# feifeibear/long-context-attention

Measured on AMD Instinct MI355X. Metric: attention TFLOP/s (algorithmic, causal fwd+bwd) + iter ms of LongContextAttention at seqlen 64K, ulysses x ring, higher is better.
Workload: dtype bf16

## Files before the change

long-context-attention_amd/csrc/usp_flash_bwd_dq64.hip:

```cpp
#include "usp_bwd_params.hpp"
#include "usp_host.hpp"
#include "usp_mfma64.hpp"

namespace usp {

#ifndef USP_Q64_PF
#define USP_Q64_PF 3
#endif
constexpr int kQ64_PF = USP_Q64_PF;
#ifndef USP_Q64_Y1
#define USP_Q64_Y1 24
#endif
constexpr int kQ64_Y1 = USP_Q64_Y1;

#ifdef USP_Q64_TIMING
#define USP_TM(...) __VA_ARGS__
#else
#define USP_TM(...)
#endif

template <int DT, bool CAUSAL>
__global__ __launch_bounds__(256, 1) void flash_bwd_dq64_kernel(const BwdParams ) {
  using E = Elem<DT>;
  using M = M64<DT>;
  constexpr int D = 128, kBM = 256;
  constexpr int ROWB = D * 2;
  constexpr int TILEB = kTile * ROWB;
  constexpr int VOFF = 2 * TILEB;
  constexpr int NKT = D / 16, NDJ = D / 32;
  constexpr int PF = kQ64_PF;

  extern __shared__ __attribute__((aligned(16))) char smem_raw[];
  if ((uint32_t)(uintptr_t)(USP_LDS char*)smem_raw != 0u) __builtin_trap();
  USP_LDS char* smem = (USP_LDS char*)(uintptr_t)0;

  const int tid = threadIdx.x;
  const int lane = tid & 63;
  const int wave = __builtin_amdgcn_readfirstlane(tid >> 6);
  const int l31 = lane & 31;
  const int hi = lane >> 5;
  typedef const __attribute__((address_space(4))) BwdParams* KArgs;
  KArgs p = (KArgs)__builtin_amdgcn_kernarg_segment_ptr();
  asm volatile("" : "+s"(p));

  const int dma_row = lane >> 4;
  const int dma_c8 = ((lane & 15) ^ ((lane >> 4) << 2)) * 16;
  const int k_voff = dma_row * (int)p->k_ss * 2 + dma_c8, v_voff = dma_row * (int)p->v_ss * 2 + dma_c8;
  const int rd_base = l31 * ROWB + ((hi ^ tile_swz<D>(l31)) * 16);
  int tr_addr[NDJ][2];
  {
    const int i = lane & 15, grp = (lane >> 4) & 1;
#pragma unroll
    for (int dj = 0; dj < NDJ; ++dj)
#pragma unroll
      for (int e = 0; e < 2; ++e) {
        const int rr = 8 * e + 4 * hi + (i >> 2);
        const int slot = 4 * dj + 2 * grp + ((i & 3) >> 1);
        tr_addr[dj][e] = rr * ROWB + ((slot ^ tile_swz<D>(rr)) * 16) + (i & 1) * 8;
      }
  }
  const float c = p->scale_log2;

  const ItemWalk walk(p->n_items);
  for (int pass = 0;; ++pass) {
  int w = walk.at(pass);
  if (w < 0) break;
  asm volatile("" : "+s"(p));
  USP_TM(const uint64_t tm_item = __builtin_amdgcn_s_memtime();)
  w = walk.dealt(w, p->nblk);
  if (p->ksplit <= 1) w = walk.grouped(w, p->nblk, p->walk_g);
  const int qt_r = w % p->nblk;
  int rest = w / p->nblk;
  const int qt = CAUSAL ? (p->nblk - 1 - qt_r) : qt_r;
  int cut = 0;
  if (p->ksplit > 1) { cut = rest % p->ksplit; rest /= p->ksplit; }
  const int h = rest % p->Hq, b = rest / p->Hq;
  const int hkv = h / p->G;
  const int q0 = qt * kBM;
  const int qw = q0 + wave * 64;
  const int off = p->causal_off;

  int blk_kv_end = p->Sk, wave_kv_end = p->Sk;
  if (CAUSAL) {
    const int blk_last = (q0 + kBM < p->Sq ? q0 + kBM : p->Sq) - 1;
    const int wav_last = (qw + 64 < p->Sq ? qw + 64 : p->Sq) - 1;
    blk_kv_end = blk_last + off + 1 < p->Sk ? blk_last + off + 1 : p->Sk;
    wave_kv_end = wav_last + off + 1 < p->Sk ? wav_last + off + 1 : p->Sk;
  }
  if (qw >= p->Sq) wave_kv_end = 0;
  const int nt = blk_kv_end > 0 ? (blk_kv_end + kTile - 1) / kTile : 0;
  int n_full = p->Sk / kTile;
// ... 31 lines not shown
                 "global_load_dwordx4 %12, %17, off offset:128\n\tglobal_load_dwordx4 %13, %17, off offset:160\n\t"
                 "global_load_dwordx4 %14, %17, off offset:192\n\tglobal_load_dwordx4 %15, %17, off offset:224\n\t"
                 "s_waitcnt vmcnt(0)"
                 : "=&a"(qf[qb][0]), "=&a"(qf[qb][1]), "=&a"(qf[qb][2]), "=&a"(qf[qb][3]), "=&a"(qf[qb][4]), "=&a"(qf[qb][5]),
                   "=&a"(qf[qb][6]), "=&a"(qf[qb][7]), "=&a"(df[qb][0]), "=&a"(df[qb][1]), "=&a"(df[qb][2]), "=&a"(df[qb][3]),
                   "=&a"(df[qb][4]), "=&a"(df[qb][5]), "=&a"(df[qb][6]), "=&a"(df[qb][7])
                 : "v"(qp), "v"(dp) : "memory");
#endif
    const float lse = p->lse[b * p->lse_sb + h * p->lse_sh + row_c];
    const float dlt = p->delta[b * p->dl_sb + h * p->dl_sh + row_c];
    const bool live = row < p->Sq && lse != USP_NEG_INF;
    nl[qb] = live ? -lse * kLog2e : USP_NEG_INF;
    dl[qb] = live ? dlt : 0.f;
  }

  const int k_rowb = (int)p->k_ss * 2, v_rowb = (int)p->v_ss * 2;
  const int64_t k_tb = (int64_t)kTile * k_rowb, v_tb = (int64_t)kTile * v_rowb;
  int k_step = 4 * k_rowb - 1024, v_step = 4 * v_rowb - 1024;
  int lds_w = wave * 4096;
  const char* k_cur = p->k + 2 * (b * p->k_sb + hkv * p->k_sh) + (int64_t)wave * 16 * k_rowb + tb * k_tb;
  const char* v_cur = p->v + 2 * (b * p->v_sb + hkv * p->v_sh) + (int64_t)wave * 16 * v_rowb + tb * v_tb;
  int rows_kv = p->Sk - 16 * wave - tb * kTile;
  u32x4 k_rs, v_rs;
  int dma_buf = 0;
  auto dma_open = [&](int buf) {
    k_rs = make_rsrc_rows(k_cur, rows_kv, 16, k_rowb, 2 * D);
    v_rs = make_rsrc_rows(v_cur, rows_kv, 16, v_rowb, 2 * D);
    dma_buf = buf;
    k_cur += k_tb;
    v_cur += v_tb;
    rows_kv -= kTile;
  };
  auto dma_piece = [&](int n) {
    asm volatile("" : "+s"(lds_w), "+s"(k_step), "+s"(v_step));
    const int i = n & 3;
    if (n < 4) lds_dma16_asm(k_rs, lds_w + dma_buf * TILEB, k_voff ^ (16 * i), i * k_step, i);
    else lds_dma16_asm(v_rs, lds_w + VOFF + dma_buf * TILEB, v_voff ^ (16 * i), i * v_step, i);
  };

  f32x16 dq[2][NDJ];
#pragma unroll
  for (int qb = 0; qb < 2; ++qb)
#pragma unroll
    for (int dj = 0; dj < NDJ; ++dj) {
#pragma unroll
      for (int r = 0; r < 16; ++r) dq[qb][dj][r] = 0.f;
      pin_agpr(dq[qb][dj]);
    }

  dma_open(tb & 1);
#pragma unroll
  for (int n = 0; n < 8; ++n) dma_piece(n);
  dma_drain();
  __syncthreads();

  auto iter = [&](auto mask_c, int t, bool work) __attribute__((always_inline)) {
    constexpr bool MASK = decltype(mask_c)::value;
    const int par = t & 1;
    if (work) {
#pragma unroll
      for (int qb = 0; qb < 2; ++qb)
#pragma unroll
        for (int kt = 0; kt < NKT; ++kt) { pin_agpr4(qf[qb][kt]); pin_agpr4(df[qb][kt]); }
      int kr = rd_base + par * TILEB, vr = rd_base + VOFF + par * TILEB;
      asm volatile("" : "+v"(kr), "+v"(vr));
      USP_LDS const char* kt_base = smem + par * TILEB;
      f32x16 bs[2][2], bd[2][2];
      u32x4 pk[2][4];
      u32x4 ka[2 * NKT], va[2 * NKT], xa[4 * NDJ];
      auto rd_k = [&](int f) { ka[f] = *(USP_LDS const u32x4*)(smem + (f & 1) * 32 * ROWB + (kr ^ (32 * (f >> 1)))); };
      auto rd_v = [&](int f) { va[f] = *(USP_LDS const u32x4*)(smem + (f & 1) * 32 * ROWB + (vr ^ (32 * (f >> 1)))); };
      auto rd_x = [&](int f) {
        USP_LDS const char* xb = kt_base + (f / NDJ) * 16 * ROWB;
        const u32x2 a0 = lds_read_tr16(xb + tr_addr[f % NDJ][0]);
        const u32x2 a1 = lds_read_tr16(xb + tr_addr[f % NDJ][1]);
        xa[f] = u32x4{a0[0], a0[1], a1[0], a1[1]};
      };
      auto X = [&](int qb, int n) {
        const int ks = n >> 3, kb = ks >> 1, r = 8 * (ks & 1) + (n & 7);
        bs[qb][kb][r] = fast_exp2(__builtin_fmaf(bs[qb][kb][r], c, nl[qb]));
      };
      auto Y = [&](int qb, int n) {
        const int ks = n >> 3, kb = ks >> 1, r = 8 * (ks & 1) + (n & 7);
        bd[qb][kb][r] = (bd[qb][kb][r] - dl[qb]) * bs[qb][kb][r];
        if (r & 1) pk[qb][ks][(n & 7) >> 1] = E::pack2(bd[qb][kb][r - 1], bd[qb][kb][r]);
      };
      auto mask = [&](int qb) {
        const int row = qw + 32 * qb + l31;
        int klim = p->Sk - 1;
        if (CAUSAL) klim = row + off < klim ? row + off : klim;
        const int kb0 = t * kTile + 4 * hi;
#pragma unroll
        for (int r = 0; r < 16; ++r) {
          const int key = kb0 + (r & 3) + 8 * (r >> 2);
          if (key > klim) bs[qb][0][r] = USP_NEG_INF;
          if (key + 32 > klim) bs[qb][1][r] = USP_NEG_INF;
        }
      };
#pragma unroll
      for (int f = 0; f < PF; ++f) rd_k(f);
      __builtin_amdgcn_sched_barrier(0);
#pragma unroll
      for (int i = 0; i < 16; ++i) {
        const int kt = i >> 1, kb = i & 1;
        if (kt == 0) M::template s_first<MASK>(bs[0][kb], ka[i], qf[0][0]);
        else M::template s_next<MASK>(bs[0][kb], ka[i], qf[0][kt]);
        if (i == 0) { __builtin_amdgcn_sched_barrier(0); dma_open(par ^ 1); }
        if (i + PF < 16) rd_k(i + PF);
        if (i >= 1 && i <= 8) dma_piece(i - 1);
        __builtin_amdgcn_sched_barrier(0);
      }
      if (MASK) { mfma_settle(bs[0]); mask(0); }
#pragma unroll
      for (int i = 0; i < 16; ++i) {
        const int kt = i >> 1, kb = i & 1;
        if (kt == 0) M::template s_first<MASK>(bs[1][kb], ka[i], qf[1][0]);
        else M::template s_next<MASK>(bs[1][kb], ka[i], qf[1][kt]);
        if (i == 0) __builtin_amdgcn_sched_barrier(0);
        X(0, 2 * i); X(0, 2 * i + 1);
        if (i >= 16 - PF) rd_v(i - (16 - PF));
        __builtin_amdgcn_sched_barrier(0);
      }
      if (MASK) { mfma_settle(bs[1]); mask(1); }
#pragma unroll
      for (int i = 0; i < 16; ++i) {
        const int kt = i >> 1, kb = i & 1;
        if (kt == 0) M::template s_first<MASK>(bd[0][kb], va[i], df[0][0]);
        else M::template s_next<MASK>(bd[0][kb], va[i], df[0][kt]);
        if (i == 0) __builtin_amdgcn_sched_barrier(0);
        if (i + PF < 16) rd_v(i + PF);
        X(1, 2 * i); X(1, 2 * i + 1);
        __builtin_amdgcn_sched_barrier(0);
      }
#pragma unroll
      for (int i = 0; i < 16; ++i) {
        const int kt = i >> 1, kb = i & 1;
        if (kt == 0) M::template s_first<MASK>(bd[1][kb], va[i], df[1][0]);
        else M::template s_next<MASK>(bd[1][kb], va[i], df[1][kt]);
        if (i == 0) __builtin_amdgcn_sched_barrier(0);
        Y(0, 2 * i); Y(0, 2 * i + 1);
        if (i >= 16 - PF) rd_x(i - (16 - PF));
        __builtin_amdgcn_sched_barrier(0);
      }
      constexpr int NY1 = kQ64_Y1;
      static_assert(NY1 >= 16 && NY1 <= 28, "dS of k-step ks must be packed before gap 16 + 4 ks");
#pragma unroll
      for (int i = 0; i < 16; ++i) {
        M::template o_acc<MASK>(dq[0][i % NDJ], xa[i], pk[0][i / NDJ]);
        if (i == 0) __builtin_amdgcn_sched_barrier(0);
        if (i + PF < 16) rd_x(i + PF);
#pragma unroll
        for (int n = i * 32 / NY1; n < (i + 1) * 32 / NY1; ++n) Y(1, n);
        __builtin_amdgcn_sched_barrier(0);
      }
#pragma unroll
      for (int i = 0; i < 16; ++i) {
        M::template o_acc<MASK>(dq[1][i % NDJ], xa[i], pk[1][i / NDJ]);
        if (16 + i < NY1) {
#pragma unroll
          for (int n = (16 + i) * 32 / NY1; n < (16 + i + 1) * 32 / NY1; ++n) Y(1, n);
        }
        __builtin_amdgcn_sched_barrier(0);
      }
    } else {
      dma_open(par ^ 1);
#pragma unroll
      for (int n = 0; n < 8; ++n) dma_piece(n);
    }
    dma_drain();
    __syncthreads();
  };
  const std::integral_constant<bool, false> plain;
  const std::integral_constant<bool, true> masked;
  int t = tb;
  USP_TM(const uint64_t tm_loop = __builtin_amdgcn_s_memtime();)
  __builtin_amdgcn_s_waitcnt(0x0f70);
  for (; t < e_full; ++t) iter(plain, t, true);
  __builtin_amdgcn_s_waitcnt(0x0f70);
  for (; t < e_own; ++t) iter(masked, t, true);
  mfma_settle(dq);
  USP_TM(const uint64_t tm_own = __builtin_amdgcn_s_memtime(); const uint64_t tm_plain_n = n_full;)
  for (; t < te; ++t) iter(plain, t, false);
  USP_TM(const uint64_t tm_epi = __builtin_amdgcn_s_memtime();)

  mfma_settle(dq);
  asm volatile("" : "+s"(p));
  const bool wide = (p->wide16 & 1) != 0;
#pragma unroll
  for (int qb = 0; qb < 2; ++qb) {
    const int row = qw + 32 * qb + l31;
    if (wide) {
      const int row_c = row < p->Sq ? row : 0;
      store_row16_wide<E, NDJ>(p->dq16 + 2 * (b * p->dq16_sb + (int64_t)row_c * p->dq16_ss + h * p->dq16_sh), dq[qb], p->scale, hi,
                               row < p->Sq);
    } else if (row < p->Sq) {
      float* o1 = p->dq + b * p->dq_sb + (int64_t)row * p->dq_ss + h * p->dq_sh;
      char* h1 = p->dq16 ? p->dq16 + 2 * (b * p->dq16_sb + (int64_t)row * p->dq16_ss + h * p->dq16_sh) : nullptr;
      int acc_f = p->accum_dq;
      if (p->ksplit > 1) {
        o1 = p->ws_dq + ((((int64_t)cut * p->B + b) * p->Sq + row) * p->Hq + h) * D;
        h1 = nullptr;
        acc_f = 0;
      }
      const float sc = p->scale;
#pragma unroll
      for (int dj = 0; dj < NDJ; ++dj)
#pragma unroll
        for (int g4 = 0; g4 < 4; ++g4) {
          const int d0 = 32 * dj + 8 * g4 + 4 * hi;
          f32x4 v1 = {dq[qb][dj][4 * g4] * sc, dq[qb][dj][4 * g4 + 1] * sc, dq[qb][dj][4 * g4 + 2] * sc,
                      dq[qb][dj][4 * g4 + 3] * sc};
          if (acc_f) v1 += *(const f32x4*)(o1 + d0);
          if (h1) *(u32x2*)(h1 + 2 * d0) = u32x2{E::pack2(v1[0], v1[1]), E::pack2(v1[2], v1[3])};
          else *(f32x4*)(o1 + d0) = v1;
        }
    }
  }
  __syncthreads();
USP_TM(
  if (pass < 3 && lane == 0 && (blockIdx.x % 61) == 0)
    printf("TQ wg %3d pass %d wave %d qt %2d tiles own %3d (plain %3d) wg %3d : prologue %6llu own tiles %8llu (%5llu / tile) idle %6llu epilogue %6llu\n",
           (int)blockIdx.x, pass, wave, qt, n_w, (int)tm_plain_n, nt, (unsigned long long)(tm_loop - tm_item),
           (unsigned long long)(tm_own - tm_loop), (unsigned long long)((tm_own - tm_loop) / (n_w > 0 ? n_w : 1)),
           (unsigned long long)(tm_epi - tm_own), (unsigned long long)(__builtin_amdgcn_s_memtime() - tm_epi));
)
  }
}

bool dq64_serves(const BwdParams& p_in) {
  if (p_in.seq_q || p_in.seq_k || p_in.sched || p_in.win_on) return false;
  if ((p_in.k_ss * 2) % 256 != 0 || (p_in.v_ss * 2) % 256 != 0 || p_in.k_ss * 128 >= (1LL << 31) || p_in.v_ss * 128 >= (1LL << 31))
    return false;
  return true;
}

bool launch_dq64(const BwdParams& p_in, int dtype, bool causal, hipStream_t st, int* rc) {
  if (!dq64_serves(p_in)) return false;
  BwdParams p = p_in;
  p.nblk = (p.Sq + 255) / 256;
  p.n_items = p.B * p.Hq * p.nblk * p.ksplit;
  p.wide16 = (p.ksplit <= 1 && p.dq16 && !p.accum_dq && tensor_aligned(p.dq16, p.dq16_sb, p.dq16_ss, p.dq16_sh, 16, 8)) ? 1 : 0;
  const int grid = persistent_grid(p.n_items, device_cus(), p.interleave);
  const size_t lds = 4 * kTile * 128 * 2;
  with_dtype_causal(dtype, causal, [&](auto dt, auto c) {
    hipLaunchKernelGGL((flash_bwd_dq64_kernel<decltype(dt)::value, decltype(c)::value>), dim3(grid), dim3(256), lds, st, p);
  });
  *rc = launched();
  return true;
}

}
```

long-context-attention_amd/csrc/usp_flash_fwd64.hip:

```cpp
#include "usp_fwd_params.hpp"
#include "usp_host.hpp"
#include "usp_mfma64.hpp"

namespace usp {

#ifndef USP_F64_NEA
#define USP_F64_NEA 42
#endif
constexpr int kF64_NEA = USP_F64_NEA;
#ifndef USP_F64_LEAD
#define USP_F64_LEAD 2
#endif
constexpr int kF64_LEAD = USP_F64_LEAD;
#ifndef USP_F64_PFK
#define USP_F64_PFK 2
#endif
constexpr int kF64_PFK = USP_F64_PFK;
#ifndef USP_F64_PFV
#define USP_F64_PFV 2
#endif
constexpr int kF64_PFV = USP_F64_PFV;
#ifndef USP_F64_MAX0
#define USP_F64_MAX0 22
#endif
constexpr int kF64_MAX0 = USP_F64_MAX0;
#ifndef USP_F64_DMA0
#define USP_F64_DMA0 2
#endif
constexpr int kF64_DMA0 = USP_F64_DMA0;
#ifndef USP_F64_DMAS
#define USP_F64_DMAS 6
#endif
constexpr int kF64_DMAS = USP_F64_DMAS;

#ifdef USP_F64_TIMING
#define USP_TM(...) __VA_ARGS__
#else
#define USP_TM(...)
#endif

template <int DT, bool CAUSAL, bool SPLIT = false>
__global__ __launch_bounds__(256, 1) void flash_fwd64_kernel(const FwdArgsT<SPLIT> ) {
  using E = Elem<DT>;
  using M = M64<DT>;
  constexpr int D = 128;
  constexpr int kBM = 256;
  constexpr int ROWB = D * 2;
  constexpr int KBYTES = kBN * ROWB;
  constexpr int NKT = D / 16;
  constexpr int NDJ = D / 32;
  constexpr int VOFF = 2 * KBYTES;

  extern __shared__ __attribute__((aligned(16))) char smem_raw[];
  USP_LDS char* smem = (USP_LDS char*)smem_raw;

  const int tid = threadIdx.x;
  const int lane = tid & 63;
  const int wave = __builtin_amdgcn_readfirstlane(tid >> 6);
  const int l31 = lane & 31;
  const int hi = lane >> 5;
  typedef const __attribute__((address_space(4))) FwdArgsT<SPLIT>* KArgs;
  KArgs p = (KArgs)__builtin_amdgcn_kernarg_segment_ptr();
  asm volatile("" : "+s"(p));

  const int k_voff = (16 * wave + (lane >> 4)) * (int)p->k_ss * 2 + (((lane & 15) ^ (lane >> 4)) * 16);
  const int v_voff = (16 * wave + ((lane & 15) >> 2)) * (int)p->v_ss * 2 + (32 * (lane >> 4) + 8 * (lane & 3)) * 2;
  const int k_rd = l31 * ROWB + ((hi ^ (l31 & 15)) * 16);
  const int v_rd = VOFF + hi * NDJ * 256 + ((lane & 15) >> 2) * 64 + ((lane >> 4) & 1) * 32 + (lane & 3) * 8;
  const float c = p->scale_log2;

  const ItemWalk walk(p->n_items);
  for (int pass = 0;; ++pass) {
  int w = walk.at(pass);
  if (w < 0) break;
// ... 32 lines not shown
    off -= kb;
  }
  auto n_keys = [&]() { if constexpr (SPLIT) return sk_cut; else return p->Sk; };

  int blk_kv_end = n_keys(), wave_kv_end = n_keys();
  if (CAUSAL) {
    const int blk_last = (q0 + kBM < p->Sq ? q0 + kBM : p->Sq) - 1;
    const int wav_last = (qw + 64 < p->Sq ? qw + 64 : p->Sq) - 1;
    blk_kv_end = blk_last + off + 1 < n_keys() ? blk_last + off + 1 : n_keys();
    wave_kv_end = wav_last + off + 1 < n_keys() ? wav_last + off + 1 : n_keys();
  }
  if (qw >= p->Sq) wave_kv_end = 0;
  const int nt = blk_kv_end > 0 ? (blk_kv_end + kBN - 1) / kBN : 0;
  int n_full = n_keys() / kBN;
  if (CAUSAL) {
    const int lim = qw + off + 1;
    const int nf = lim > 0 ? lim / kBN : 0;
    n_full = nf < n_full ? nf : n_full;
  }
  if (n_full > nt) n_full = nt;

USP_TM(
  const uint64_t tm_item = __builtin_amdgcn_s_memtime();
)
  u32x4 qf[2][NKT];
#pragma unroll
  for (int qb = 0; qb < 2; ++qb) {
    const int row = qw + 32 * qb + l31;
    const int row_c = row < p->Sq ? row : p->Sq - 1;
    const char* qp = p->q + 2 * (b * p->q_sb + (int64_t)row_c * p->q_ss + h * p->q_sh) + 16 * hi;
#pragma unroll
    for (int t = 0; t < NKT; ++t) qf[qb][t] = *(const u32x4*)(qp + 32 * t);
  }
#pragma unroll
  for (int qb = 0; qb < 2; ++qb)
#pragma unroll
    for (int t = 0; t < NKT; ++t) pin_agpr4(qf[qb][t]);

  const int64_t k_tb = (int64_t)kBN * p->k_ss * 2, v_tb = (int64_t)kBN * p->v_ss * 2;
  const char* k_cur = p->k + 2 * (b * p->k_sb + hkv * p->k_sh);
  const char* v_cur = p->v + 2 * (b * p->v_sb + hkv * p->v_sh);
  if constexpr (SPLIT) { k_cur += 2 * (int64_t)kb * p->k_ss; v_cur += 2 * (int64_t)kb * p->v_ss; }
  int rows_kv = n_keys();
  const int k_rowb = (int)p->k_ss * 2, v_rowb = (int)p->v_ss * 2;
  int lds_w = wave * 4096, k_step = 4 * (int)p->k_ss * 2 - 1024, v_step = 4 * (int)p->v_ss * 2 - 1024;
  u32x4 k_rs, v_rs;
  int k_ahead = 0;
  int dma_kbuf = 0, dma_vbuf = 0;
  auto dma_open = [&](int kbuf, int vbuf) {
    k_rs = make_rsrc_rows(k_cur, rows_kv + kBN * k_ahead, kBN, k_rowb, 2 * D);
    v_rs = make_rsrc_rows(v_cur, rows_kv, kBN, v_rowb, 2 * D);
    k_cur += k_tb;
    v_cur += v_tb;
    rows_kv -= kBN;
    dma_kbuf = kbuf; dma_vbuf = vbuf;
  };
  auto dma_open_k = [&](int kbuf) {
    k_rs = make_rsrc_rows(k_cur, rows_kv, kBN, k_rowb, 2 * D);
    k_cur += k_tb;
    k_ahead = -1;
    dma_kbuf = kbuf;
  };
  auto dma_piece = [&](int n) {
    asm volatile("" : "+s"(lds_w), "+s"(k_step), "+s"(v_step));
    if (n < 4) lds_dma16_asm(k_rs, lds_w + dma_kbuf * KBYTES, k_voff ^ (64 * n), n * k_step, n);
    else lds_dma16_asm(v_rs, lds_w + VOFF + dma_vbuf * KBYTES, v_voff, (n - 4) * v_step, n - 4);
  };
  auto dma_all = [&](int kbuf, int vbuf) {
    dma_open(kbuf, vbuf);
#pragma unroll
    for (int n = 0; n < 8; ++n) dma_piece(n);
  };

  f32x16 o[2][NDJ];
#pragma unroll
  for (int qb = 0; qb < 2; ++qb)
#pragma unroll
    for (int dj = 0; dj < NDJ; ++dj) {
#pragma unroll
      for (int r = 0; r < 16; ++r) o[qb][dj][r] = 0.f;
      pin_agpr(o[qb][dj]);
    }
  float m_run[2] = {USP_NEG_INF, USP_NEG_INF};
  float l_run[2] = {0.f, 0.f};

  auto qk = [&](int kbuf, f32x16 (&s)[2][2]) {
#pragma unroll
    for (int kt = 0; kt < NKT; ++kt) {
      USP_LDS const char* kp = smem + kbuf * KBYTES + (k_rd ^ (32 * kt));
      const u32x4 k0 = *(USP_LDS const u32x4*)kp;
      const u32x4 k1 = *(USP_LDS const u32x4*)(kp + 32 * ROWB);
#pragma unroll
      for (int qb = 0; qb < 2; ++qb) {
        if (kt == 0) { M::template s_first<true>(s[qb][0], k0, qf[qb][0]); M::template s_first<true>(s[qb][1], k1, qf[qb][0]); }
        else { M::template s_next<true>(s[qb][0], k0, qf[qb][kt]); M::template s_next<true>(s[qb][1], k1, qf[qb][kt]); }
      }
    }
    mfma_settle(s);
  };
  auto mask = [&](int kt0, f32x16 (&s)[2][2]) {
#pragma unroll
    for (int qb = 0; qb < 2; ++qb) {
      const int row = qw + 32 * qb + l31;
      int klim = n_keys() - 1;
      if (CAUSAL) klim = row + off < klim ? row + off : klim;
      const int kb0 = kt0 + 4 * hi;
#pragma unroll
      for (int r = 0; r < 16; ++r) {
        const int key = kb0 + (r & 3) + 8 * (r >> 2);
        if (key > klim) s[qb][0][r] = USP_NEG_INF;
        if (key + 32 > klim) s[qb][1][r] = USP_NEG_INF;
      }
    }
  };
  f32x16 sa[2][2], sb[2][2];
#pragma unroll
  for (int qb = 0; qb < 2; ++qb)
#pragma unroll
    for (int kb = 0; kb < 2; ++kb)
#pragma unroll
      for (int r = 0; r < 16; ++r) { sa[qb][kb][r] = 0.f; sb[qb][kb][r] = 0.f; }
  dma_all(0, 0);
  dma_open_k(1);
#pragma unroll
  for (int n = 0; n < 4; ++n) dma_piece(n);
  dma_drain();
  __syncthreads();
  if (nt > 0 && wave_kv_end > 0) qk(0, sa);
  __syncthreads();

  constexpr float kThr = 8.f;
  constexpr int NA = 32, NB = 32;
  constexpr int NEA = kF64_NEA, LEAD = kF64_LEAD, PFK = kF64_PFK, PFV = kF64_PFV, MAX0 = kF64_MAX0;
  constexpr int DMA0 = kF64_DMA0, DMAS = kF64_DMAS;
  static_assert(64 - NEA <= 22, "k-step 3 of P must be complete two slots before slot 24 of phase B");
  static_assert(MAX0 >= 1 && MAX0 < NB && DMAS >= 1 && DMA0 + 7 * DMAS < NA + NB, "");
  const float thr_raw = kThr / c;
  float m_thr[2] = {USP_NEG_INF, USP_NEG_INF};
  float nmc[2] = {0.f, 0.f};
  auto first_ref = [&](const float (&mt_lane)[2]) {
#pragma unroll
    for (int qb = 0; qb < 2; ++qb) {
      const float m_new = xhalf_max(mt_lane[qb]);
      const float m_use = (m_new == USP_NEG_INF) ? 0.f : m_new;
      m_run[qb] = m_new;
      m_thr[qb] = m_new + thr_raw;
      nmc[qb] = -(m_use * c);
    }
  };
  auto rescale = [&](const float (&mt_lane)[2]) {
    asm volatile("; rescale (rare)" ::: "memory");
    mfma_settle(o);
#pragma unroll
    for (int qb = 0; qb < 2; ++qb) {
      const float m_new = fmaxf(m_run[qb], xhalf_max(mt_lane[qb]));
      const float m_use = (m_new == USP_NEG_INF) ? 0.f : m_new;
// ... 9 lines not shown
    }
#pragma unroll
    for (int qb = 0; qb < 2; ++qb)
#pragma unroll
      for (int dj = 0; dj < NDJ; ++dj) pin_agpr(o[qb][dj]);
    operand_settle();
  };
  auto decide = [&](f32x16 (&s)[2][2]) {
    float mt[2];
#pragma unroll
    for (int qb = 0; qb < 2; ++qb) {
      mt[qb] = s[qb][0][0];
#pragma unroll
      for (int r = 1; r < 16; ++r) mt[qb] = fmaxf(mt[qb], s[qb][0][r]);
#pragma unroll
      for (int r = 0; r < 16; ++r) mt[qb] = fmaxf(mt[qb], s[qb][1][r]);
    }
    first_ref(mt);
  };
  auto iter = [&](auto par_c, auto mode_c, int jpar, int kt0_next, f32x16 (&cs)[2][2], f32x16 (&ns)[2][2])
      __attribute__((always_inline)) {
    constexpr int PARV = decltype(par_c)::value, MODE = decltype(mode_c)::value;
    const int par = PARV < 2 ? PARV : jpar;
    dma_open(par, par ^ 1);
    auto dma_slot = [&](int g) {
      if (g >= DMA0 && (g - DMA0) % DMAS == 0 && (g - DMA0) / DMAS < 8) dma_piece((g - DMA0) / DMAS);
    };
    USP_LDS const char* kb = smem + (par ^ 1) * KBYTES;
    USP_LDS const char* vb = smem + par * KBYTES + v_rd;
    int kr = k_rd;
    asm volatile("" : "+v"(kr));
    u32x4 ka[2 * NKT];
    auto rd_k = [&](int f) {
      ka[f] = *(USP_LDS const u32x4*)(kb + (f & 1) * 32 * ROWB + (kr ^ (32 * (f >> 1))));
    };
    u32x4 va[4 * NDJ];
    auto rd_v = [&](int f) {
      USP_LDS const char* vp = vb + (4 * (f / NDJ) * NDJ + (f % NDJ)) * 256;
      const u32x2 v0 = lds_read_tr16(vp);
      const u32x2 v1 = lds_read_tr16(vp + 2 * NDJ * 256);
      va[f] = u32x4{v0[0], v0[1], v1[0], v1[1]};
    };
    float rs[2] = {0.f, 0.f};
    u32x4 pf[2][4];
    auto get = [&](int e) -> float { return cs[(e >> 3) & 1][e >> 5][8 * ((e >> 4) & 1) + (e & 7)]; };
    auto consume = [&](int e) {
      rs[(e >> 3) & 1] += get(e);
      if (e & 1) pf[(e >> 3) & 1][e >> 4][(e & 7) >> 1] = E::pack2(get(e - 1), get(e));
    };
    auto exp_elem = [&](int e) {
      cs[(e >> 3) & 1][e >> 5][8 * ((e >> 4) & 1) + (e & 7)] = fast_exp2(__builtin_fmaf(get(e), c, nmc[(e >> 3) & 1]));
      if (e > 0) consume(e - 1);
      if (e == 63) consume(63);
    };
    if (MODE != 2) {
#pragma unroll
      for (int f = 0; f < PFK; ++f) rd_k(f);
    }
#pragma unroll
    for (int e = 0; e < LEAD; ++e) exp_elem(e);
    __builtin_amdgcn_sched_barrier(0);
#pragma unroll
    for (int sl = 0; sl < NA; ++sl) {
      const int f = sl >> 1, kt = f >> 1, kbk = f & 1, qb = sl & 1;
      if (MODE != 2) {
        if (qb == 0 && f + PFK < 2 * NKT) rd_k(f + PFK);
        if (kt == 0) M::template s_first<MODE != 0>(ns[qb][kbk], ka[f], qf[qb][0]);
        else M::template s_next<MODE != 0>(ns[qb][kbk], ka[f], qf[qb][kt]);
      }
#pragma unroll
      for (int e = LEAD + sl * (NEA - LEAD) / NA; e < LEAD + (sl + 1) * (NEA - LEAD) / NA; ++e) exp_elem(e);
      if (sl >= NA - 2 * PFV && ((sl - (NA - 2 * PFV)) & 1) == 0) rd_v((sl - (NA - 2 * PFV)) >> 1);
      dma_slot(sl);
      __builtin_amdgcn_sched_barrier(0);
    }
    if (MODE == 1) {
      mfma_settle(ns);
      mask(kt0_next, ns);
    }
    float mt[2] = {USP_NEG_INF, USP_NEG_INF};
    bool keep = true;
    constexpr int NMAX = NB - MAX0;
#pragma unroll
    for (int i = 0; i < NB; ++i) {
      const int f = i >> 1, qb = i & 1;
      if (qb == 0 && f + PFV < 4 * NDJ) rd_v(f + PFV);
      M::template o_acc<MODE != 0>(o[qb][f % NDJ], va[f], pf[qb][f / NDJ]);
      if (NEA + i < 64) exp_elem(NEA + i);
      if (i == 64 - NEA - 1 || (NEA == 64 && i == 0)) { l_run[0] += rs[0]; l_run[1] += rs[1]; }
      if (MODE != 2 && i >= MAX0) {
#pragma unroll
        for (int x = (i - MAX0) * 64 / NMAX; x < (i - MAX0 + 1) * 64 / NMAX; ++x)
          mt[x >> 5] = fmaxf(mt[x >> 5], ns[x >> 5][(x >> 4) & 1][x & 15]);
        if (i == NB - 1) keep = __all(mt[0] <= m_thr[0] && mt[1] <= m_thr[1]);
      }
      dma_slot(NA + i);
      __builtin_amdgcn_sched_barrier(0);
    }
    if (!keep) rescale(mt);
    dma_drain();
    __syncthreads();
  };

  const int n_w = wave_kv_end > 0 ? (wave_kv_end + kBN - 1) / kBN : 0;
  if (n_full > n_w) n_full = n_w;
  int j = 0;
USP_TM(
  const uint64_t tm_loop = __builtin_amdgcn_s_memtime();
  uint64_t tm_hot = tm_loop;
)
  if (n_w > 0) {
    if (n_full == 0) mask(0, sa);
    decide(sa);
    const std::integral_constant<int, 0> c0;
    const std::integral_constant<int, 1> c1;
    const std::integral_constant<int, 2> c2;
    const int n_hot = n_full - 1;
    for (; j + 1 < n_hot; j += 2) {
      iter(c0, c0, 0, 0, sa, sb);
      iter(c1, c0, 1, 0, sb, sa);
    }
    auto adopt = [&]() {
#pragma unroll
      for (int qb = 0; qb < 2; ++qb)
#pragma unroll
        for (int kb = 0; kb < 2; ++kb) sa[qb][kb] = sb[qb][kb];
    };
USP_TM(
    tm_hot = __builtin_amdgcn_s_memtime();
)
    if (j < n_hot) { iter(c0, c0, 0, 0, sa, sb); adopt(); ++j; }
    for (; j < n_w; ++j) {
      if (j + 1 >= n_w) iter(c2, c2, j & 1, 0, sa, sb);
      else { iter(c2, c1, j & 1, (j + 1) * kBN, sa, sb); adopt(); }
    }
  }
USP_TM(
  const uint64_t tm_own = __builtin_amdgcn_s_memtime();
)
  for (; j < nt; ++j) {
    dma_all(j & 1, (j + 1) & 1);
    dma_drain();
    __syncthreads();
  }

USP_TM(
  const uint64_t tm_idle = __builtin_amdgcn_s_memtime();
)
  mfma_settle(o);
  asm volatile("" : "+s"(p));
#pragma unroll
  for (int qb = 0; qb < 2; ++qb) {
    const int row = qw + 32 * qb + l31;
    const float l_tot = xhalf_sum(l_run[qb]);
    const bool empty = !(l_tot > 0.f);
    const float inv = empty ? 0.f : 1.f / l_tot;
    const float blk_lse = empty ? USP_NEG_INF : (m_run[qb] * c + log2f(l_tot)) * kLn2;
    float w_blk = inv, w_old = 0.f, new_lse = blk_lse;
    float* lse_p = p->lse + b * p->lse_sb + h * p->lse_sh + row;
    if constexpr (SPLIT) lse_p += (int64_t)ks * p->B * p->Hq * p->Sq;
    const bool valid = row < p->Sq;
    const bool fin = row >= p->final_begin && row < p->final_end;
    const bool wide = !p->merge_in && p->out_wide && __all(!valid || fin);
    if (valid) {
// ... 37 lines not shown
          for (int g4 = 0; g4 < 4; ++g4) {
            const int d0 = 32 * dj + 8 * g4 + 4 * hi;
            f32x4 val = {o[qb][dj][4 * g4] * w_blk, o[qb][dj][4 * g4 + 1] * w_blk, o[qb][dj][4 * g4 + 2] * w_blk,
                         o[qb][dj][4 * g4 + 3] * w_blk};
            if (p->merge_in) {
              const f32x4 a = *(const f32x4*)(p->acc + arow + d0);
              val += a * w_old;
            }
            if (fin) {
              u32x2 pk = {E::pack2(val[0], val[1]), E::pack2(val[2], val[3])};
              *(u32x2*)(p->out + 2 * (orow + d0)) = pk;
            } else {
              *(f32x4*)(p->acc + arow + d0) = val;
            }
          }
        }
      }
    }
  }
USP_TM(
  {
    const uint64_t tm_end = __builtin_amdgcn_s_memtime();
    if (lane == 0 && (blockIdx.x % 61) == 0 && pass < 4)
      printf("TF wg %3d pass %d wave %d qt %2d tiles own %3d wg %3d : prologue %6llu hot-loop %8llu (%5llu / tile) tail-tiles %6llu idle %6llu epilogue %6llu\n",
             (int)blockIdx.x, pass, wave, qt, n_w, nt, (unsigned long long)(tm_loop - tm_item), (unsigned long long)(tm_hot - tm_loop),
             (unsigned long long)((tm_hot - tm_loop) / (n_full > 2 ? (n_full - 1) / 2 * 2 : 1)), (unsigned long long)(tm_own - tm_hot),
             (unsigned long long)(tm_idle - tm_own), (unsigned long long)(tm_end - tm_idle));
  }
)
  }
}

template <bool SPLIT>
static int launch64(FwdArgsT<SPLIT>& p, int dtype, bool causal, hipStream_t st) {
  p.nq = (p.Sq + 255) / 256;
  p.n_items = p.B * p.Hq * p.nq;
  if constexpr (SPLIT) p.n_items *= p.ksplit;
  const int grid = persistent_grid(p.n_items, device_cus(), p.interleave);
  const size_t lds = 2 * 2 * kBN * 128 * 2;
  with_dtype_causal(dtype, causal, [&](auto dt, auto c) {
    hipLaunchKernelGGL((flash_fwd64_kernel<decltype(dt)::value, decltype(c)::value, SPLIT>), dim3(grid), dim3(256), lds, st, p);
  });
  return launched();
}

bool launch_fwd64(const FwdArgsT<true>& p_in, int dtype, bool causal, hipStream_t st, int* rc) {
  if ((p_in.k_ss * 2) % 256 != 0 || p_in.k_ss * 128 >= (1LL << 31) || p_in.v_ss * 128 >= (1LL << 31)) return false;
  if (p_in.win_on || p_in.seq_q) return false;
  if (p_in.ksplit > 1) {
    FwdArgsT<true> p = p_in;
    p.acc = p.ws_o;
    p.a_sb = (int64_t)p.Sq * p.Hq * 128; p.a_ss = (int64_t)p.Hq * 128; p.a_sh = 128;
    p.lse = p.ws_lse;
    p.lse_sb = (int64_t)p.Hq * p.Sq; p.lse_sh = p.Sq;
    p.merge_in = 0; p.final_begin = 0; p.final_end = 0; p.out_wide = 0;
    *rc = launch64(p, dtype, causal, st);
    if (*rc == USP_OK) *rc = launch_split_merge(p_in, dtype, 128, st);
  } else {
    FwdArgsT<false> p;
    static_cast<FwdParams&>(p) = p_in;
    *rc = launch64(p, dtype, causal, st);
  }
// ... 5 lines not shown
```

Before: 1015.

## Triple-buffer K tiles in LDS and prefetch next K fragments across iterations

Both the forward and dq-backward 64-row kernels move from two to three K buffers in LDS, so the K tile two steps ahead is DMA'd while the next one sits ready. The first K fragments of the next tile are read into registers at the end of the current iteration, replacing per-phase PF-depth prefetch with grouped reads followed by explicit LDS waitcnts. The aim is to take LDS read latency at the head of each QK phase off the critical path. In exchange the kernels use more LDS and hold K fragments in registers across iterations, and new timing probes are added under USP_TM.

```diff
diff --git a/long-context-attention_amd/csrc/usp_flash_bwd_dq64.hip b/long-context-attention_amd/csrc/usp_flash_bwd_dq64.hip
--- a/long-context-attention_amd/csrc/usp_flash_bwd_dq64.hip
+++ b/long-context-attention_amd/csrc/usp_flash_bwd_dq64.hip
@@ -4,10 +4,6 @@
 
 namespace usp {
 
-#ifndef USP_Q64_PF
-#define USP_Q64_PF 3
-#endif
-constexpr int kQ64_PF = USP_Q64_PF;
 #ifndef USP_Q64_Y1
 #define USP_Q64_Y1 24
 #endif
@@ -26,9 +22,8 @@
   constexpr int D = 128, kBM = 256;
   constexpr int ROWB = D * 2;
   constexpr int TILEB = kTile * ROWB;
-  constexpr int VOFF = 2 * TILEB;
+  constexpr int VOFF = 3 * TILEB;
   constexpr int NKT = D / 16, NDJ = D / 32;
-  constexpr int PF = kQ64_PF;
 
   extern __shared__ __attribute__((aligned(16))) char smem_raw[];
   if ((uint32_t)(uintptr_t)(USP_LDS char*)smem_raw != 0u) __builtin_trap();
@@ -66,7 +61,7 @@
   int w = walk.at(pass);
   if (w < 0) break;
   asm volatile("" : "+s"(p));
-  USP_TM(const uint64_t tm_item = __builtin_amdgcn_s_memtime();)
+  USP_TM(const uint64_t tm_item = __builtin_amdgcn_s_memtime(); uint64_t tm_last = 0, tm_body = 0, tm_lds = 0, tm_drain = 0, tm_bar = 0;)
   w = walk.dealt(w, p->nblk);
   if (p->ksplit <= 1) w = walk.grouped(w, p->nblk, p->walk_g);
   const int qt_r = w % p->nblk;
@@ -144,20 +139,27 @@
   const char* v_cur = p->v + 2 * (b * p->v_sb + hkv * p->v_sh) + (int64_t)wave * 16 * v_rowb + tb * v_tb;
   int rows_kv = p->Sk - 16 * wave - tb * kTile;
   u32x4 k_rs, v_rs;
-  int dma_buf = 0;
-  auto dma_open = [&](int buf) {
-    k_rs = make_rsrc_rows(k_cur, rows_kv, 16, k_rowb, 2 * D);
+  int k_ahead = 0;
+  int dma_kb = 0, dma_vb = 0;
+  auto dma_open = [&](int kb, int vb) {
+    k_rs = make_rsrc_rows(k_cur, rows_kv + kTile * k_ahead, 16, k_rowb, 2 * D);
     v_rs = make_rsrc_rows(v_cur, rows_kv, 16, v_rowb, 2 * D);
-    dma_buf = buf;
+    dma_kb = kb; dma_vb = vb;
     k_cur += k_tb;
     v_cur += v_tb;
     rows_kv -= kTile;
   };
+  auto dma_open_k = [&](int kb) {
+    k_rs = make_rsrc_rows(k_cur, rows_kv, 16, k_rowb, 2 * D);
+    k_cur += k_tb;
+    k_ahead = -1;
+    dma_kb = kb;
+  };
   auto dma_piece = [&](int n) {
     asm volatile("" : "+s"(lds_w), "+s"(k_step), "+s"(v_step));
     const int i = n & 3;
-    if (n < 4) lds_dma16_asm(k_rs, lds_w + dma_buf * TILEB, k_voff ^ (16 * i), i * k_step, i);
-    else lds_dma16_asm(v_rs, lds_w + VOFF + dma_buf * TILEB, v_voff ^ (16 * i), i * v_step, i);
+    if (n < 4) lds_dma16_asm(k_rs, lds_w + dma_kb, k_voff ^ (16 * i), i * k_step, i);
+    else lds_dma16_asm(v_rs, lds_w + VOFF + dma_vb, v_voff ^ (16 * i), i * v_step, i);
   };
 
   f32x16 dq[2][NDJ];
@@ -170,26 +172,38 @@
       pin_agpr(dq[qb][dj]);
     }
 
-  dma_open(tb & 1);
+  int ks_cur = (tb % 3) * TILEB;
+  int ks_nxt = ks_cur == 2 * TILEB ? 0 : ks_cur + TILEB;
+  int ks_dma = ks_nxt == 2 * TILEB ? 0 : ks_nxt + TILEB;
+  dma_open(ks_cur, (tb & 1) * TILEB);
 #pragma unroll
   for (int n = 0; n < 8; ++n) dma_piece(n);
+  dma_open_k(ks_nxt);
+#pragma unroll
+  for (int n = 0; n < 4; ++n) dma_piece(n);
   dma_drain();
   __syncthreads();
+  u32x4 ka[2 * NKT];
+  {
+    int kr = rd_base + ks_cur;
+#pragma unroll
+    for (int f = 0; f < 2 * NKT; ++f) ka[f] = *(USP_LDS const u32x4*)(smem + (f & 1) * 32 * ROWB + (kr ^ (32 * (f >> 1))));
+  }
 
   auto iter = [&](auto mask_c, int t, bool work) __attribute__((always_inline)) {
     constexpr bool MASK = decltype(mask_c)::value;
-    const int par = t & 1;
+    const int vb = (t & 1) * TILEB;
     if (work) {
 #pragma unroll
       for (int qb = 0; qb < 2; ++qb)
 #pragma unroll
         for (int kt = 0; kt < NKT; ++kt) { pin_agpr4(qf[qb][kt]); pin_agpr4(df[qb][kt]); }
-      int kr = rd_base + par * TILEB, vr = rd_base + VOFF + par * TILEB;
+      int kr = rd_base + ks_nxt, vr = rd_base + VOFF + vb;
       asm volatile("" : "+v"(kr), "+v"(vr));
-      USP_LDS const char* kt_base = smem + par * TILEB;
+      USP_LDS const char* kt_base = smem + ks_cur;
       f32x16 bs[2][2], bd[2][2];
       u32x4 pk[2][4];
-      u32x4 ka[2 * NKT], va[2 * NKT], xa[4 * NDJ];
+      u32x4 va[2 * NKT], xa[4 * NDJ];
       auto rd_k = [&](int f) { ka[f] = *(USP_LDS const u32x4*)(smem + (f & 1) * 32 * ROWB + (kr ^ (32 * (f >> 1)))); };
       auto rd_v = [&](int f) { va[f] = *(USP_LDS const u32x4*)(smem + (f & 1) * 32 * ROWB + (vr ^ (32 * (f >> 1)))); };
       auto rd_x = [&](int f) {
@@ -220,15 +234,11 @@
         }
       };
 #pragma unroll
-      for (int f = 0; f < PF; ++f) rd_k(f);
-      __builtin_amdgcn_sched_barrier(0);
-#pragma unroll
       for (int i = 0; i < 16; ++i) {
         const int kt = i >> 1, kb = i & 1;
         if (kt == 0) M::template s_first<MASK>(bs[0][kb], ka[i], qf[0][0]);
         else M::template s_next<MASK>(bs[0][kb], ka[i], qf[0][kt]);
-        if (i == 0) { __builtin_amdgcn_sched_barrier(0); dma_open(par ^ 1); }
-        if (i + PF < 16) rd_k(i + PF);
+        if (i == 0) { __builtin_amdgcn_sched_barrier(0); dma_open(ks_dma, vb ^ TILEB); }
         if (i >= 1 && i <= 8) dma_piece(i - 1);
         __builtin_amdgcn_sched_barrier(0);
       }
@@ -240,17 +250,19 @@
         else M::template s_next<MASK>(bs[1][kb], ka[i], qf[1][kt]);
         if (i == 0) __builtin_amdgcn_sched_barrier(0);
         X(0, 2 * i); X(0, 2 * i + 1);
-        if (i >= 16 - PF) rd_v(i - (16 - PF));
+        rd_v(i);
         __builtin_amdgcn_sched_barrier(0);
       }
       if (MASK) { mfma_settle(bs[1]); mask(1); }
+      USP_TM(const uint64_t tw0 = __builtin_amdgcn_s_memtime();)
+      __builtin_amdgcn_s_waitcnt(0xc07f);
+      USP_TM(const uint64_t tw1 = __builtin_amdgcn_s_memtime();)
 #pragma unroll
       for (int i = 0; i < 16; ++i) {
         const int kt = i >> 1, kb = i & 1;
         if (kt == 0) M::template s_first<MASK>(bd[0][kb], va[i], df[0][0]);
         else M::template s_next<MASK>(bd[0][kb], va[i], df[0][kt]);
         if (i == 0) __builtin_amdgcn_sched_barrier(0);
-        if (i + PF < 16) rd_v(i + PF);
         X(1, 2 * i); X(1, 2 * i + 1);
         __builtin_amdgcn_sched_barrier(0);
       }
@@ -261,16 +273,18 @@
         else M::template s_next<MASK>(bd[1][kb], va[i], df[1][kt]);
         if (i == 0) __builtin_amdgcn_sched_barrier(0);
         Y(0, 2 * i); Y(0, 2 * i + 1);
-        if (i >= 16 - PF) rd_x(i - (16 - PF));
-        __builtin_amdgcn_sched_barrier(0);
-      }
+        rd_x(i);
+        __builtin_amdgcn_sched_barrier(0);
+      }
+      USP_TM(const uint64_t tw2 = __builtin_amdgcn_s_memtime();)
+      __builtin_amdgcn_s_waitcnt(0xc07f);
+      USP_TM(const uint64_t tw3 = __builtin_amdgcn_s_memtime();)
       constexpr int NY1 = kQ64_Y1;
       static_assert(NY1 >= 16 && NY1 <= 28, "dS of k-step ks must be packed before gap 16 + 4 ks");
 #pragma unroll
       for (int i = 0; i < 16; ++i) {
         M::template o_acc<MASK>(dq[0][i % NDJ], xa[i], pk[0][i / NDJ]);
         if (i == 0) __builtin_amdgcn_sched_barrier(0);
-        if (i + PF < 16) rd_x(i + PF);
 #pragma unroll
         for (int n = i * 32 / NY1; n < (i + 1) * 32 / NY1; ++n) Y(1, n);
         __builtin_amdgcn_sched_barrier(0);
@@ -282,23 +296,32 @@
 #pragma unroll
           for (int n = (16 + i) * 32 / NY1; n < (16 + i + 1) * 32 / NY1; ++n) Y(1, n);
         }
-        __builtin_amdgcn_sched_barrier(0);
-      }
+        rd_k(i);
+        __builtin_amdgcn_sched_barrier(0);
+      }
+      USP_TM(const uint64_t tw4 = __builtin_amdgcn_s_memtime();)
+      __builtin_amdgcn_s_waitcnt(0xc07f);
+      USP_TM(tm_lds += (tw1 - tw0) + (tw3 - tw2) + (__builtin_amdgcn_s_memtime() - tw4);)
     } else {
-      dma_open(par ^ 1);
+      dma_open(ks_dma, vb ^ TILEB);
 #pragma unroll
       for (int n = 0; n < 8; ++n) dma_piece(n);
     }
+    { const int k0 = ks_cur; ks_cur = ks_nxt; ks_nxt = ks_dma; ks_dma = k0; }
+    USP_TM(const uint64_t tm0 = __builtin_amdgcn_s_memtime();)
     dma_drain();
+    USP_TM(const uint64_t tm1 = __builtin_amdgcn_s_memtime();)
     __syncthreads();
+    USP_TM(const uint64_t tm2 = __builtin_amdgcn_s_memtime();
+           if (work) { tm_body += tm0 - tm_last; tm_drain += tm1 - tm0; tm_bar += tm2 - tm1; } tm_last = tm2;)
   };
   const std::integral_constant<bool, false> plain;
   const std::integral_constant<bool, true> masked;
   int t = tb;
-  USP_TM(const uint64_t tm_loop = __builtin_amdgcn_s_memtime();)
-  __builtin_amdgcn_s_waitcnt(0x0f70);
+  USP_TM(const uint64_t tm_loop = __builtin_amdgcn_s_memtime(); tm_last = tm_loop;)
+  __builtin_amdgcn_s_waitcnt(0x0070);
   for (; t < e_full; ++t) iter(plain, t, true);
-  __builtin_amdgcn_s_waitcnt(0x0f70);
+  __builtin_amdgcn_s_waitcnt(0x0070);
   for (; t < e_own; ++t) iter(masked, t, true);
   mfma_settle(dq);
   USP_TM(const uint64_t tm_own = __builtin_amdgcn_s_memtime(); const uint64_t tm_plain_n = n_full;)
@@ -341,9 +364,11 @@
   __syncthreads();
 USP_TM(
   if (pass < 3 && lane == 0 && (blockIdx.x % 61) == 0)
-    printf("TQ wg %3d pass %d wave %d qt %2d tiles own %3d (plain %3d) wg %3d : prologue %6llu own tiles %8llu (%5llu / tile) idle %6llu epilogue %6llu\n",
+    printf("TQ wg %3d pass %d wave %d qt %2d tiles own %3d (plain %3d) wg %3d : prologue %6llu own tiles %8llu (%5llu / tile: blocks %5llu of which LDS waits %4llu, drain %4llu, barrier %4llu) idle %6llu epilogue %6llu\n",
            (int)blockIdx.x, pass, wave, qt, n_w, (int)tm_plain_n, nt, (unsigned long long)(tm_loop - tm_item),
            (unsigned long long)(tm_own - tm_loop), (unsigned long long)((tm_own - tm_loop) / (n_w > 0 ? n_w : 1)),
+           (unsigned long long)(tm_body / (n_w > 0 ? n_w : 1)), (unsigned long long)(tm_lds / (n_w > 0 ? n_w : 1)),
+           (unsigned long long)(tm_drain / (n_w > 0 ? n_w : 1)), (unsigned long long)(tm_bar / (n_w > 0 ? n_w : 1)),
            (unsigned long long)(tm_epi - tm_own), (unsigned long long)(__builtin_amdgcn_s_memtime() - tm_epi));
 )
   }
@@ -363,7 +388,7 @@
   p.n_items = p.B * p.Hq * p.nblk * p.ksplit;
   p.wide16 = (p.ksplit <= 1 && p.dq16 && !p.accum_dq && tensor_aligned(p.dq16, p.dq16_sb, p.dq16_ss, p.dq16_sh, 16, 8)) ? 1 : 0;
   const int grid = persistent_grid(p.n_items, device_cus(), p.interleave);
-  const size_t lds = 4 * kTile * 128 * 2;
+  const size_t lds = 5 * kTile * 128 * 2;
   with_dtype_causal(dtype, causal, [&](auto dt, auto c) {
     hipLaunchKernelGGL((flash_bwd_dq64_kernel<decltype(dt)::value, decltype(c)::value>), dim3(grid), dim3(256), lds, st, p);
   });
diff --git a/long-context-attention_amd/csrc/usp_flash_fwd64.hip b/long-context-attention_amd/csrc/usp_flash_fwd64.hip
--- a/long-context-attention_amd/csrc/usp_flash_fwd64.hip
+++ b/long-context-attention_amd/csrc/usp_flash_fwd64.hip
@@ -12,14 +12,14 @@
 #define USP_F64_LEAD 2
 #endif
 constexpr int kF64_LEAD = USP_F64_LEAD;
-#ifndef USP_F64_PFK
-#define USP_F64_PFK 2
-#endif
-constexpr int kF64_PFK = USP_F64_PFK;
-#ifndef USP_F64_PFV
-#define USP_F64_PFV 2
-#endif
-constexpr int kF64_PFV = USP_F64_PFV;
+#ifndef USP_F64_GK
+#define USP_F64_GK 4
+#endif
+constexpr int kF64_GK = USP_F64_GK;
+#ifndef USP_F64_GV
+#define USP_F64_GV 4
+#endif
+constexpr int kF64_GV = USP_F64_GV;
 #ifndef USP_F64_MAX0
 #define USP_F64_MAX0 22
 #endif
@@ -49,7 +49,7 @@
   constexpr int KBYTES = kBN * ROWB;
   constexpr int NKT = D / 16;
   constexpr int NDJ = D / 32;
-  constexpr int VOFF = 2 * KBYTES;
+  constexpr int VOFF = 3 * KBYTES;
 
   extern __shared__ __attribute__((aligned(16))) char smem_raw[];
   USP_LDS char* smem = (USP_LDS char*)smem_raw;
@@ -128,6 +128,7 @@
 
 USP_TM(
   const uint64_t tm_item = __builtin_amdgcn_s_memtime();
+  uint64_t tm_last = 0, tm_body = 0, tm_lds = 0, tm_drain = 0, tm_bar = 0;
 )
   u32x4 qf[2][NKT];
 #pragma unroll
@@ -162,14 +163,14 @@
     dma_kbuf = kbuf; dma_vbuf = vbuf;
   };
   auto dma_open_k = [&](int kbuf) {
-    k_rs = make_rsrc_rows(k_cur, rows_kv, kBN, k_rowb, 2 * D);
+    k_rs = make_rsrc_rows(k_cur, rows_kv + kBN * k_ahead, kBN, k_rowb, 2 * D);
     k_cur += k_tb;
-    k_ahead = -1;
+    k_ahead -= 1;
     dma_kbuf = kbuf;
   };
   auto dma_piece = [&](int n) {
     asm volatile("" : "+s"(lds_w), "+s"(k_step), "+s"(v_step));
-    if (n < 4) lds_dma16_asm(k_rs, lds_w + dma_kbuf * KBYTES, k_voff ^ (64 * n), n * k_step, n);
+    if (n < 4) lds_dma16_asm(k_rs, lds_w + dma_kbuf, k_voff ^ (64 * n), n * k_step, n);
     else lds_dma16_asm(v_rs, lds_w + VOFF + dma_vbuf * KBYTES, v_voff, (n - 4) * v_step, n - 4);
   };
   auto dma_all = [&](int kbuf, int vbuf) {
@@ -193,7 +194,7 @@
   auto qk = [&](int kbuf, f32x16 (&s)[2][2]) {
 #pragma unroll
     for (int kt = 0; kt < NKT; ++kt) {
-      USP_LDS const char* kp = smem + kbuf * KBYTES + (k_rd ^ (32 * kt));
+      USP_LDS const char* kp = smem + kbuf + (k_rd ^ (32 * kt));
       const u32x4 k0 = *(USP_LDS const u32x4*)kp;
       const u32x4 k1 = *(USP_LDS const u32x4*)(kp + 32 * ROWB);
 #pragma unroll
@@ -219,6 +220,7 @@
       }
     }
   };
+  int ks_a = KBYTES, ks_b = 2 * KBYTES, ks_c = 0;
   f32x16 sa[2][2], sb[2][2];
 #pragma unroll
   for (int qb = 0; qb < 2; ++qb)
@@ -227,17 +229,26 @@
 #pragma unroll
       for (int r = 0; r < 16; ++r) { sa[qb][kb][r] = 0.f; sb[qb][kb][r] = 0.f; }
   dma_all(0, 0);
-  dma_open_k(1);
+  dma_open_k(ks_a);
+#pragma unroll
+  for (int n = 0; n < 4; ++n) dma_piece(n);
+  dma_open_k(ks_b);
 #pragma unroll
   for (int n = 0; n < 4; ++n) dma_piece(n);
   dma_drain();
   __syncthreads();
   if (nt > 0 && wave_kv_end > 0) qk(0, sa);
+  u32x4 ka[2 * NKT];
+#pragma unroll
+  for (int f = 0; f < kF64_GK; ++f)
+    ka[f] = *(USP_LDS const u32x4*)(smem + ks_a + (f & 1) * 32 * ROWB + (k_rd ^ (32 * (f >> 1))));
+  __builtin_amdgcn_s_waitcnt(0xc07f);
   __syncthreads();
 
   constexpr float kThr = 8.f;
   constexpr int NA = 32, NB = 32;
-  constexpr int NEA = kF64_NEA, LEAD = kF64_LEAD, PFK = kF64_PFK, PFV = kF64_PFV, MAX0 = kF64_MAX0;
+  constexpr int NEA = kF64_NEA, LEAD = kF64_LEAD, GK = kF64_GK, GV = kF64_GV, MAX0 = kF64_MAX0;
+  static_assert(GK >= 1 && GK <= 8 && (2 * NKT) % GK == 0 && GV >= 1 && GV <= 8 && (4 * NDJ) % GV == 0, "");
   constexpr int DMA0 = kF64_DMA0, DMAS = kF64_DMAS;
   static_assert(64 - NEA <= 22, "k-step 3 of P must be complete two slots before slot 24 of phase B");
   static_assert(MAX0 >= 1 && MAX0 < NB && DMAS >= 1 && DMA0 + 7 * DMAS < NA + NB, "");
@@ -293,17 +304,18 @@
       __attribute__((always_inline)) {
     constexpr int PARV = decltype(par_c)::value, MODE = decltype(mode_c)::value;
     const int par = PARV < 2 ? PARV : jpar;
-    dma_open(par, par ^ 1);
+    dma_open(ks_c, par ^ 1);
     auto dma_slot = [&](int g) {
       if (g >= DMA0 && (g - DMA0) % DMAS == 0 && (g - DMA0) / DMAS < 8) dma_piece((g - DMA0) / DMAS);
     };
-    USP_LDS const char* kb = smem + (par ^ 1) * KBYTES;
     USP_LDS const char* vb = smem + par * KBYTES + v_rd;
-    int kr = k_rd;
-    asm volatile("" : "+v"(kr));
-    u32x4 ka[2 * NKT];
+    int kr = k_rd + ks_a, kn = k_rd + ks_b;
+    asm volatile("" : "+v"(kr), "+v"(kn));
     auto rd_k = [&](int f) {
-      ka[f] = *(USP_LDS const u32x4*)(kb + (f & 1) * 32 * ROWB + (kr ^ (32 * (f >> 1))));
+      ka[f] = *(USP_LDS const u32x4*)(smem + (f & 1) * 32 * ROWB + (kr ^ (32 * (f >> 1))));
+    };
+    auto rd_kn = [&](int f) {
+      ka[f] = *(USP_LDS const u32x4*)(smem + (f & 1) * 32 * ROWB + (kn ^ (32 * (f >> 1))));
     };
     u32x4 va[4 * NDJ];
     auto rd_v = [&](int f) {
@@ -314,6 +326,11 @@
     };
     float rs[2] = {0.f, 0.f};
     u32x4 pf[2][4];
+    auto lds_wait = [&]() {
+      USP_TM(const uint64_t tw = __builtin_amdgcn_s_memtime();)
+      __builtin_amdgcn_s_waitcnt(0xc07f);
+      USP_TM(tm_lds += __builtin_amdgcn_s_memtime() - tw;)
+    };
     auto get = [&](int e) -> float { return cs[(e >> 3) & 1][e >> 5][8 * ((e >> 4) & 1) + (e & 7)]; };
     auto consume = [&](int e) {
       rs[(e >> 3) & 1] += get(e);
@@ -324,10 +341,6 @@
       if (e > 0) consume(e - 1);
       if (e == 63) consume(63);
     };
-    if (MODE != 2) {
-#pragma unroll
-      for (int f = 0; f < PFK; ++f) rd_k(f);
-    }
 #pragma unroll
     for (int e = 0; e < LEAD; ++e) exp_elem(e);
     __builtin_amdgcn_sched_barrier(0);
@@ -335,16 +348,18 @@
     for (int sl = 0; sl < NA; ++sl) {
       const int f = sl >> 1, kt = f >> 1, kbk = f & 1, qb = sl & 1;
       if (MODE != 2) {
-        if (qb == 0 && f + PFK < 2 * NKT) rd_k(f + PFK);
+        if (qb == 0 && f % GK == 0 && f > 0) lds_wait();
+        if (qb == 0 && f + GK < 2 * NKT) rd_k(f + GK);
         if (kt == 0) M::template s_first<MODE != 0>(ns[qb][kbk], ka[f], qf[qb][0]);
         else M::template s_next<MODE != 0>(ns[qb][kbk], ka[f], qf[qb][kt]);
       }
 #pragma unroll
       for (int e = LEAD + sl * (NEA - LEAD) / NA; e < LEAD + (sl + 1) * (NEA - LEAD) / NA; ++e) exp_elem(e);
-      if (sl >= NA - 2 * PFV && ((sl - (NA - 2 * PFV)) & 1) == 0) rd_v((sl - (NA - 2 * PFV)) >> 1);
+      if (sl >= NA - 2 * GV && ((sl - (NA - 2 * GV)) & 1) == 0) rd_v((sl - (NA - 2 * GV)) >> 1);
       dma_slot(sl);
       __builtin_amdgcn_sched_barrier(0);
     }
+    lds_wait();
     if (MODE == 1) {
       mfma_settle(ns);
       mask(kt0_next, ns);
@@ -355,7 +370,8 @@
 #pragma unroll
     for (int i = 0; i < NB; ++i) {
       const int f = i >> 1, qb = i & 1;
-      if (qb == 0 && f + PFV < 4 * NDJ) rd_v(f + PFV);
+      if (qb == 0 && f % GV == 0 && f > 0) lds_wait();
+      if (qb == 0 && f + GV < 4 * NDJ) rd_v(f + GV);
       M::template o_acc<MODE != 0>(o[qb][f % NDJ], va[f], pf[qb][f / NDJ]);
       if (NEA + i < 64) exp_elem(NEA + i);
       if (i == 64 - NEA - 1 || (NEA == 64 && i == 0)) { l_run[0] += rs[0]; l_run[1] += rs[1]; }
@@ -365,12 +381,19 @@
           mt[x >> 5] = fmaxf(mt[x >> 5], ns[x >> 5][(x >> 4) & 1][x & 15]);
         if (i == NB - 1) keep = __all(mt[0] <= m_thr[0] && mt[1] <= m_thr[1]);
       }
+      if (MODE != 2 && i >= NB - 2 * GK && ((i - (NB - 2 * GK)) & 1) == 0) rd_kn((i - (NB - 2 * GK)) >> 1);
       dma_slot(NA + i);
       __builtin_amdgcn_sched_barrier(0);
     }
+    lds_wait();
     if (!keep) rescale(mt);
+    { const int k0 = ks_a; ks_a = ks_b; ks_b = ks_c; ks_c = k0; }
+    USP_TM(const uint64_t tm0 = __builtin_amdgcn_s_memtime();)
     dma_drain();
+    USP_TM(const uint64_t tm1 = __builtin_amdgcn_s_memtime();)
     __syncthreads();
+    USP_TM(const uint64_t tm2 = __builtin_amdgcn_s_memtime();
+           tm_body += tm0 - tm_last; tm_drain += tm1 - tm0; tm_bar += tm2 - tm1; tm_last = tm2;)
   };
 
   const int n_w = wave_kv_end > 0 ? (wave_kv_end + kBN - 1) / kBN : 0;
@@ -379,6 +402,7 @@
 USP_TM(
   const uint64_t tm_loop = __builtin_amdgcn_s_memtime();
   uint64_t tm_hot = tm_loop;
+  tm_last = tm_loop;
 )
   if (n_w > 0) {
     if (n_full == 0) mask(0, sa);
@@ -410,7 +434,8 @@
   const uint64_t tm_own = __builtin_amdgcn_s_memtime();
 )
   for (; j < nt; ++j) {
-    dma_all(j & 1, (j + 1) & 1);
+    dma_all(ks_c, (j + 1) & 1);
+    { const int k0 = ks_a; ks_a = ks_b; ks_b = ks_c; ks_c = k0; }
     dma_drain();
     __syncthreads();
   }
@@ -494,9 +519,11 @@
   {
     const uint64_t tm_end = __builtin_amdgcn_s_memtime();
     if (lane == 0 && (blockIdx.x % 61) == 0 && pass < 4)
-      printf("TF wg %3d pass %d wave %d qt %2d tiles own %3d wg %3d : prologue %6llu hot-loop %8llu (%5llu / tile) tail-tiles %6llu idle %6llu epilogue %6llu\n",
+      printf("TF wg %3d pass %d wave %d qt %2d tiles own %3d wg %3d : prologue %6llu hot-loop %8llu (%5llu / tile); all own tiles, per tile: phases %5llu of which LDS waits %4llu, drain %4llu, barrier %4llu; tail-tiles %6llu idle %6llu epilogue %6llu\n",
              (int)blockIdx.x, pass, wave, qt, n_w, nt, (unsigned long long)(tm_loop - tm_item), (unsigned long long)(tm_hot - tm_loop),
-             (unsigned long long)((tm_hot - tm_loop) / (n_full > 2 ? (n_full - 1) / 2 * 2 : 1)), (unsigned long long)(tm_own - tm_hot),
+             (unsigned long long)((tm_hot - tm_loop) / (n_full > 2 ? (n_full - 1) / 2 * 2 : 1)),
+             (unsigned long long)(tm_body / (n_w > 0 ? n_w : 1)), (unsigned long long)(tm_lds / (n_w > 0 ? n_w : 1)),
+             (unsigned long long)(tm_drain / (n_w > 0 ? n_w : 1)), (unsigned long long)(tm_bar / (n_w > 0 ? n_w : 1)), (unsigned long long)(tm_own - tm_hot),
              (unsigned long long)(tm_idle - tm_own), (unsigned long long)(tm_end - tm_idle));
   }
 )
@@ -509,7 +536,7 @@
   p.n_items = p.B * p.Hq * p.nq;
   if constexpr (SPLIT) p.n_items *= p.ksplit;
   const int grid = persistent_grid(p.n_items, device_cus(), p.interleave);
-  const size_t lds = 2 * 2 * kBN * 128 * 2;
+  const size_t lds = 5 * kBN * 128 * 2;
   with_dtype_causal(dtype, causal, [&](auto dt, auto c) {
     hipLaunchKernelGGL((flash_fwd64_kernel<decltype(dt)::value, decltype(c)::value, SPLIT>), dim3(grid), dim3(256), lds, st, p);
   });
```

Result: no change. 1017, median of 6 (+0.2%).
